# KyanChen/RSPrompter

Measured on NVIDIA H100. Metric: images/sec, higher is better.
Workload: dtype bf16

## Files before the change

include/rsp_b200.h:

```cpp
#ifndef RSP_B200_H_
#define RSP_B200_H_

#include <stdint.h>

#ifdef __cplusplus
extern "C" {
#endif

#define RSP_ABI_VERSION 2

int rsp_abi_version(void);
const char* rsp_last_error(void);

int rsp_gemm_bf16(const void* A, int lda, const void* W, int ldw, void* out, int ldo, int M, int N,
                  int K, const float* bias, const void* residual, int ldr, int res_fp32, int res_mod,
                  const int32_t* row_map, int act, int out_fp32, void* stream);

int rsp_conv3x3_nhwc_bf16(const void* x, int B, int H, int W, int C, const void* Wt, int ldw, void* out, int ldo,
                          int N, const float* bias, const void* residual, int ldr, int res_fp32, int act,
                          int out_fp32, void* stream);
int rsp_conv3x3_geometry_ok(int B, int H, int W, int C);

int rsp_gemm_bf16_simt(const void* A, int lda, const void* W, int ldw, void* out, int ldo, int M,
                       int N, int K, const float* bias, const void* residual, int ldr, int res_fp32,
                       int res_mod, const int32_t* row_map, int act, int out_fp32, void* stream);

int rsp_vit_attention(const void* qkv, const void* rel_h, const void* rel_w, void* out, int n_seq,
                      int T, int S, int H, int hd, void* stream);
int rsp_vit_attention_scatter(const void* qkv, const void* rel_h, const void* rel_w, void* out, int n_seq, int T,
                              int Sg, int H, int hd, const int32_t* out_row_map, void* stream);

int rsp_vit_attention_simt(const void* qkv, const void* rel_h, const void* rel_w, void* out,
                           int n_seq, int T, int S, int H, int hd, void* stream);

int rsp_layernorm(const void* in, int in_fp32, int ld_in, void* out, int out_fp32, int ld_out,
                  const float* gamma, const float* beta, const int32_t* src_map, int rows_out, int C,
                  float eps, int act, void* copy_out, int ld_copy, void* stream);

int rsp_layernorm_add(const void* x, const void* res, int res_fp32, const int32_t* res_block_map,
                      int res_block_rows, const float* gamma, const float* beta, void* out, const float* pos,
                      int pos_mod, void* out_pe, long long rows, int C, float eps, void* stream);

int rsp_patchify16(const float* img, void* out, int B, int H, int W, void* stream);

int rsp_im2col_nhwc(const void* in, void* out, int B, int H, int W, int C, int KH, int KW,
                    int stride, int pad, void* stream);

int rsp_nhwc_to_nchw(const void* in, int in_fp32, float* out, int B, int HW, int C, void* stream);

int rsp_gemm_bf16_ex(const void* A, int lda, const void* W, int ldw, void* out, int ldo, int M, int N,
                     int K, const float* bias, const void* residual, int ldr, int res_fp32, int res_mod,
                     const int32_t* row_map, int act, int out_fp32, int epi_mode, const float* ln_gamma,
                     const float* ln_beta, float ln_eps, const int32_t* res_block_map,
                     int res_block_rows, const float* hyper, float* mask_out, int grid_h, int grid_w,
                     void* stream);

int rsp_gemm_upscale_masks(const void* A, int lda, const void* W, int ldw, int M, int K, const float* bias,
                           const float* hyper, int n_out, float* mask_out, int grid_h, int grid_w, void* stream);

int rsp_add_cast_bf16(const float* a, const float* b, void* out, long long n, long long b_mod,
                      void* stream);

int rsp_token_self_attention(const void* q, const void* k, const void* v, void* out, int N, int T,
                             int heads, int c, void* stream);
int rsp_t2i_attention(const void* q, const void* K, const void* V, int ldkv, const int32_t* kv_block, void* out,
                      int N, int Tq, int HW, void* stream);
// ... 153 lines not shown
```

rsprompter_b200/_lib.py:

```python
from __future__ import annotations

import ctypes
import os
import subprocess
from pathlib import Path

import torch

_PKG_DIR = Path(__file__).resolve().parent
LIB_PATH = _PKG_DIR / "librsp_b200.so"
CSRC_DIR = _PKG_DIR / "csrc"


class RspError(RuntimeError):
    """Raised when an ``rsp_*`` entry point returns a non-zero status."""


def build_library(verbose: bool = False) -> Path:
    cmd = ["make", "-C", str(CSRC_DIR), "-j", str(os.cpu_count() or 4), "all"]
    res = subprocess.run(cmd, capture_output=True, text=True)
    if res.returncode != 0:
        raise RuntimeError(f"building librsp_b200.so failed:\n{res.stdout[-4000:]}\n{res.stderr[-4000:]}")
    if verbose:
        print(res.stdout[-2000:])
    return LIB_PATH


def _load() -> ctypes.CDLL:
    if not LIB_PATH.exists():
        raise ImportError(
            f"{LIB_PATH} not found: the CUDA extension is mandatory (no fallback path). "
            "Run `python -c 'import __graft_entry__ as g; g.build()'` or `make -C rsprompter_b200/csrc`.")
    return ctypes.CDLL(str(LIB_PATH))


_lib = _load()

_vp, _i, _f = ctypes.c_void_p, ctypes.c_int, ctypes.c_float

_SIGNATURES = {
    "rsp_abi_version": ([], _i),
    "rsp_last_error": ([], ctypes.c_char_p),
    "rsp_gemm_bf16": ([_vp, _i, _vp, _i, _vp, _i, _i, _i, _i, _vp, _vp, _i, _i, _i, _vp, _i, _i, _vp], _i),
    "rsp_gemm_bf16_simt": ([_vp, _i, _vp, _i, _vp, _i, _i, _i, _i, _vp, _vp, _i, _i, _i, _vp, _i, _i, _vp], _i),
    "rsp_vit_attention": ([_vp, _vp, _vp, _vp, _i, _i, _i, _i, _i, _vp], _i),
    "rsp_vit_attention_scatter": ([_vp, _vp, _vp, _vp, _i, _i, _i, _i, _i, _vp, _vp], _i),
    "rsp_vit_attention_simt": ([_vp, _vp, _vp, _vp, _i, _i, _i, _i, _i, _vp], _i),
    "rsp_layernorm": ([_vp, _i, _i, _vp, _i, _i, _vp, _vp, _vp, _i, _i, _f, _i, _vp, _i, _vp], _i),
    "rsp_patchify16": ([_vp, _vp, _i, _i, _i, _vp], _i),
    "rsp_layernorm_add": ([_vp, _vp, _i, _vp, _i, _vp, _vp, _vp, _vp, _i, _vp, ctypes.c_longlong, _i, _f, _vp], _i),
    "rsp_im2col_nhwc": ([_vp, _vp, _i, _i, _i, _i, _i, _i, _i, _i, _vp], _i),
    "rsp_nhwc_to_nchw": ([_vp, _i, _vp, _i, _i, _i, _vp], _i),
    "rsp_cast_f32_bf16": ([_vp, _vp, ctypes.c_longlong, _vp], _i),
    "rsp_add_table_bf16": ([_vp, _vp, _vp, ctypes.c_longlong, ctypes.c_longlong, _vp], _i),
    "rsp_gemm_bf16_ex": ([_vp, _i, _vp, _i, _vp, _i, _i, _i, _i, _vp, _vp, _i, _i, _i, _vp, _i, _i,
                          _i, _vp, _vp, _f, _vp, _i, _vp, _vp, _i, _i, _vp], _i),
    "rsp_add_cast_bf16": ([_vp, _vp, _vp, ctypes.c_longlong, ctypes.c_longlong, _vp], _i),
    "rsp_token_self_attention": ([_vp, _vp, _vp, _vp, _i, _i, _i, _i, _vp], _i),
    "rsp_t2i_attention": ([_vp, _vp, _vp, _i, _vp, _vp, _i, _i, _i, _vp], _i),
    "rsp_i2t_attention": ([_vp, _vp, _vp, _vp, _vp, _i, _i, _i, _vp], _i),
    "rsp_t2i_fused": ([_vp, _i, _vp, _vp, _vp, _vp, _vp, _i, _i, _i, _vp], _i),
    "rsp_i2t_fused": ([_vp, _i, _vp, _vp, _vp, _vp, _vp, _vp, _vp, _vp, _vp, _f, _vp, _i, _i, _i, _vp], _i),
    "rsp_rpn_decode": ([_vp, _i, _vp, _i, _i, _i, _i, _i, _i, _vp, _vp, _f, _f, _f, _i, _i, _vp, _vp, _vp], _i),
    "rsp_bbox_cls_decode": ([_vp, _i, _vp, _i, _vp, _vp, _i, _i, _vp, _f, _f, _f, _vp, _vp, _vp, _vp], _i),
    "rsp_rpn_decode_shapes": ([_vp, _i, _vp, _i, _i, _i, _i, _i, _i, _vp, _vp, _vp, _f, _i, _i, _vp, _vp, _vp], _i),
    "rsp_nms_batched_topk": ([_vp, _vp, _vp, _i, _i, _f, _vp, _vp, _vp, _i, _vp], _i),
    "rsp_bbox_cls_decode_shapes": ([_vp, _i, _vp, _i, _vp, _vp, _i, _i, _vp, _vp, _f, _vp, _vp, _vp, _vp], _i),
    "rsp_nms_batched": ([_vp, _vp, _vp, _i, _i, _f, _vp, _vp, _vp, _vp], _i),
    "rsp_compact_keep": ([_vp, _vp, _vp, _vp, _i, _i, _i, _vp, _vp, _vp, _vp, _vp, _vp], _i),
    "rsp_soft_nms_workspace_bytes": ([_i, _i, _i, _vp], _i),
    "rsp_soft_nms_batched": ([_vp, _vp, _vp, _vp, _i, _i, _i, _f, _f, _f, _i, _i, _i, _vp, ctypes.c_size_t, _vp, _vp,
                              _vp, _vp, _vp, _vp], _i),
    "rsp_roi_align_nhwc": ([_vp, _vp, _vp, _vp, _vp, _i, _vp, _i, _i, _i, _f, _vp, _vp], _i),
    "rsp_mask_paste": ([_vp, _vp, _i, _i, _i, _i, _i, _f, _i, _vp], _i),
    "rsp_pool2_nhwc": ([_vp, _vp, _i, _i, _i, _i, _i, _vp], _i),
    "rsp_zero_border_nhwc": ([_vp, _i, _i, _i, _i, _vp], _i),
    "rsp_sigmoid_f32": ([_vp, _vp, ctypes.c_longlong, _vp], _i),
    "rsp_mask_paste_boxes": ([_vp, _vp, _vp, _i, _i, _i, _i, _i, _f, _i, _vp], _i),
    "rsp_groupnorm_nhwc": ([_vp, _vp, _vp, _vp, _vp, _vp, _i, _i, _i, _i, _i, _f, _i, _vp], _i),
    "rsp_ms_deform_attn_sample": ([_vp, _vp, _i, _vp, _vp, _i, _i, _i, _i, _vp, _vp], _i),
# ... 1146 lines not shown
```

rsprompter_b200/csrc/abi.cu:

```cuda
#include "../../include/rsp_b200.h"

#include "attention.h"
#include "gemm.h"
#include "rowops.h"

namespace rsp { const char* last_error(); }
using namespace rsp;

static inline cudaStream_t S(void* s) { return static_cast<cudaStream_t>(s); }

extern "C" {

int rsp_abi_version(void) { return RSP_ABI_VERSION; }
const char* rsp_last_error(void) { return rsp::last_error(); }

static GemmArgs make_gemm_args(const void* A, int lda, const void* W, int ldw, void* out, int ldo,
                               int M, int N, int K, const float* bias, const void* residual, int ldr,
                               int res_fp32, int res_mod, const int32_t* row_map, int act,
                               int out_fp32) {
  GemmArgs a;
  a.A = A; a.lda = lda; a.W = W; a.ldw = ldw; a.out = out; a.ldo = ldo;
  a.M = M; a.N = N; a.K = K; a.bias = bias; a.residual = residual; a.ldr = ldr;
  a.res_fp32 = res_fp32; a.res_mod = res_mod; a.row_map = row_map; a.act = act;
  a.out_fp32 = out_fp32;
// ... 23 lines not shown
  return conv3x3_bf16(a, S(stream));
}

int rsp_conv3x3_geometry_ok(int B, int H, int W, int C) { return conv3x3_geometry_ok(B, H, W, C) ? 1 : 0; }

int rsp_gemm_bf16_simt(const void* A, int lda, const void* W, int ldw, void* out, int ldo, int M,
                       int N, int K, const float* bias, const void* residual, int ldr, int res_fp32,
                       int res_mod, const int32_t* row_map, int act, int out_fp32, void* stream) {
  return gemm_bf16_simt(make_gemm_args(A, lda, W, ldw, out, ldo, M, N, K, bias, residual, ldr,
                                       res_fp32, res_mod, row_map, act, out_fp32), S(stream));
}

static AttentionArgs make_att_args(const void* qkv, const void* rel_h, const void* rel_w, void* out,
                                   int n_seq, int T, int Sg, int H, int hd, const int32_t* out_row_map = nullptr) {
  AttentionArgs a;
  a.qkv = qkv; a.rel_h = rel_h; a.rel_w = rel_w; a.out = out;
  a.n_seq = n_seq; a.T = T; a.S = Sg; a.H = H; a.hd = hd; a.out_row_map = out_row_map;
  return a;
}

int rsp_vit_attention(const void* qkv, const void* rel_h, const void* rel_w, void* out, int n_seq,
                      int T, int Sg, int H, int hd, void* stream) {
  return vit_attention(make_att_args(qkv, rel_h, rel_w, out, n_seq, T, Sg, H, hd), S(stream));
}

int rsp_vit_attention_scatter(const void* qkv, const void* rel_h, const void* rel_w, void* out, int n_seq, int T,
                              int Sg, int H, int hd, const int32_t* out_row_map, void* stream) {
  return vit_attention(make_att_args(qkv, rel_h, rel_w, out, n_seq, T, Sg, H, hd, out_row_map), S(stream));
}

int rsp_vit_attention_simt(const void* qkv, const void* rel_h, const void* rel_w, void* out,
                           int n_seq, int T, int Sg, int H, int hd, void* stream) {
  return vit_attention_simt(make_att_args(qkv, rel_h, rel_w, out, n_seq, T, Sg, H, hd), S(stream));
}

int rsp_attn_softmax_bias(const float* scores, int lds, const float* tab, int ldt, int NT, void* P, int ldp, int n_rows,
                          int T, int Sg, float scale, void* stream) {
  return attn_softmax_bias(scores, lds, tab, ldt, NT, P, ldp, n_rows, T, Sg, scale, S(stream));
}

int rsp_transpose_cols(const void* in, int ld, int col0, int C, int n_seq, int T, void* out, void* stream) {
  return transpose_cols(in, ld, col0, C, n_seq, T, out, S(stream));
}

int rsp_split_heads(const void* in, int ld, int col0, int H, int hd, int n_seq, int T, void* out, void* stream) {
  return split_heads(in, ld, col0, H, hd, n_seq, T, out, S(stream));
}

int rsp_layernorm(const void* in, int in_fp32, int ld_in, void* out, int out_fp32, int ld_out,
                  const float* gamma, const float* beta, const int32_t* src_map, int rows_out, int C,
                  float eps, int act, void* copy_out, int ld_copy, void* stream) {
  LayerNormArgs a;
  a.copy_out = copy_out; a.ld_copy = ld_copy;
  a.in = in; a.in_fp32 = in_fp32; a.ld_in = ld_in; a.out = out; a.out_fp32 = out_fp32;
  a.ld_out = ld_out; a.gamma = gamma; a.beta = beta; a.src_map = src_map; a.rows_out = rows_out;
  a.C = C; a.eps = eps; a.act = act;
  return layernorm_rows(a, S(stream));
}

int rsp_layernorm_add(const void* x, const void* res, int res_fp32, const int32_t* res_block_map,
                      int res_block_rows, const float* gamma, const float* beta, void* out, const float* pos,
                      int pos_mod, void* out_pe, long long rows, int C, float eps, void* stream) {
  return layernorm_add(x, res, res_fp32, res_block_map, res_block_rows, gamma, beta, out, pos, pos_mod, out_pe, rows,
                       C, eps, S(stream));
}

// ... 344 lines not shown
```

rsprompter_b200/csrc/attention.cu:

```cuda
#include <cstdlib>

#include "attention.h"
#include "sm90.cuh"

namespace rsp {

constexpr float LOG2E = 1.4426950408889634f;

__device__ __forceinline__ float fast_exp2(float x) {
  float y;
  asm("ex2.approx.ftz.f32 %0, %1;" : "=f"(y) : "f"(x));
  return y;
}
__device__ __forceinline__ uint32_t pack_f16x2(float lo, float hi) {
  __half2 v = __floats2half2_rn(lo, hi);
  return *reinterpret_cast<uint32_t*>(&v);
}
__device__ __forceinline__ uint32_t bf16x2_to_f16x2(uint32_t w) {
  return pack_f16x2(__uint_as_float(w << 16), __uint_as_float(w & 0xffff0000u));
}

template <int HD, int S>
struct AttCfg {
  static constexpr int T = S * S;
// ... 344 lines not shown
  const uint64_t tstr[1] = {static_cast<uint64_t>(HD) * 2};
  const uint32_t qbox[3] = {64, C::BM, 1}, qbox_t[3] = {16, C::BM, 1};
  const uint32_t kvbox[3] = {64, C::BN, 1}, kvbox_t[3] = {16, C::BN, 1};
  const uint32_t tbox[2] = {64, static_cast<uint32_t>(C::NTAB)}, tbox_t[2] = {16, static_cast<uint32_t>(C::NTAB)};
  CUtensorMap tq, tkv, th, tw, tq_t, tkv_t, th_t, tw_t;
  RSP_TRY(make_tmap_swizzled(&tq, a.qkv, 3, qdims, qstr, qbox, 0, 128));
  RSP_TRY(make_tmap_swizzled(&tkv, a.qkv, 3, qdims, qstr, kvbox, 0, 128));
  RSP_TRY(make_tmap_swizzled(&th, a.rel_h, 2, tdims, tstr, tbox, 0, 128));
  RSP_TRY(make_tmap_swizzled(&tw, a.rel_w, 2, tdims, tstr, tbox, 0, 128));
  if (C::TAIL > 0) {
    RSP_TRY(make_tmap_swizzled(&tq_t, a.qkv, 3, qdims, qstr, qbox_t, 0, 32));
    RSP_TRY(make_tmap_swizzled(&tkv_t, a.qkv, 3, qdims, qstr, kvbox_t, 0, 32));
    RSP_TRY(make_tmap_swizzled(&th_t, a.rel_h, 2, tdims, tstr, tbox_t, 0, 32));
    RSP_TRY(make_tmap_swizzled(&tw_t, a.rel_w, 2, tdims, tstr, tbox_t, 0, 32));
  } else {
    tq_t = tq; tkv_t = tkv; th_t = th; tw_t = tw;
  }
  auto kern = vit_attention_kernel<HD, S>;
  static bool attr_set_dev[kMaxDevices] = {};
  bool& attr_set = attr_set_dev[current_device()];
  if (!attr_set) {
    RSP_CHECK_CUDA(cudaFuncSetAttribute(kern, cudaFuncAttributeMaxDynamicSharedMemorySize, C::SMEM_BYTES));
    attr_set = true;
  }
  const long long items = static_cast<long long>(a.n_seq) * a.H * C::NQT;
  RSP_CHECK_ARG(items > 0 && items < (1ll << 31), "attention: %lld query tiles", items);
  p.n_items = static_cast<int>(items);
  const int grid = static_cast<int>(items < num_sms() ? items : num_sms());
  kern<<<grid, 384, C::SMEM_BYTES, stream>>>(tq, tq_t, tkv, tkv_t, th, th_t, tw, tw_t, p);
  RSP_CHECK_LAUNCH();
  return RSP_OK;
}

int vit_attention(const AttentionArgs& a, cudaStream_t stream) {
  RSP_CHECK_ARG(a.qkv && a.rel_h && a.rel_w && a.out, "attention: null pointer");
  RSP_CHECK_ARG(a.T == a.S * a.S, "attention: T=%d is not S^2 (S=%d)", a.T, a.S);
  RSP_CHECK_ARG(a.n_seq > 0 && a.H > 0, "attention: bad n_seq/H");
  if (a.S != 14 && a.S != 32 && a.S != 64)
    return vit_attention_simt(a, stream);
  if (a.hd == 64) {
    if (a.S == 64) return launch_att<64, 64>(a, stream);
    if (a.S == 32) return launch_att<64, 32>(a, stream);
    return launch_att<64, 14>(a, stream);
  }
  if (a.hd == 80) {
    if (a.S == 64) return launch_att<80, 64>(a, stream);
    if (a.S == 32) return launch_att<80, 32>(a, stream);
    return launch_att<80, 14>(a, stream);
  }
  set_last_error("attention: head dim %d unsupported (64, 80)", a.hd);
  return RSP_ERR_UNSUPPORTED;
}

__global__ void vit_attention_simt_kernel(const __nv_bfloat16* __restrict__ qkv,
                                          const __nv_bfloat16* __restrict__ rel_h,
                                          const __nv_bfloat16* __restrict__ rel_w,
                                          __nv_bfloat16* __restrict__ out, int T, int S, int H,
                                          int hd, float scale, const int* __restrict__ out_row_map) {
  const int D = H * hd;
  const int tq = blockIdx.x * blockDim.x + threadIdx.x;
  const int head = blockIdx.y;
  const int seq = blockIdx.z;
  if (tq >= T) return;
  const int qh = tq / S, qw = tq % S;
  const __nv_bfloat16* qp = qkv + (static_cast<size_t>(seq) * T + tq) * 3 * D + head * hd;
  float q[128];
  for (int d = 0; d < hd; ++d) q[d] = __bfloat162float(qp[d]);
  float rh[128], rw[128];
  for (int k = 0; k < S; ++k) {
    float ah = 0.f, aw = 0.f;
    const __nv_bfloat16* th = rel_h + static_cast<size_t>(qh - k + S - 1) * hd;
    const __nv_bfloat16* tw = rel_w + static_cast<size_t>(qw - k + S - 1) * hd;
    for (int d = 0; d < hd; ++d) {
      ah += q[d] * __bfloat162float(th[d]);
      aw += q[d] * __bfloat162float(tw[d]);
    }
    rh[k] = ah; rw[k] = aw;
  }
  float m = -INFINITY, l = 0.f;
  float o[128];
  for (int d = 0; d < hd; ++d) o[d] = 0.f;
  for (int k = 0; k < T; ++k) {
// ... 33 lines not shown
```

rsprompter_b200/csrc/attention.h:

```cpp
#pragma once
#include "host_util.h"

namespace rsp {

struct AttentionArgs {
  const void* qkv = nullptr;
  const void* rel_h = nullptr;
  const void* rel_w = nullptr;
  void* out = nullptr;
  int n_seq = 0;
  int T = 0;
  int S = 0;
  int H = 0;
  int hd = 0;
  const int* out_row_map = nullptr;
};

int vit_attention(const AttentionArgs& a, cudaStream_t stream);
int vit_attention_simt(const AttentionArgs& a, cudaStream_t stream);
int attn_softmax_bias(const float* scores, int lds, const float* tab, int ldt, int NT, void* P, int ldp, int n_rows,
                      int T, int S, float scale, cudaStream_t stream);
int transpose_cols(const void* in, int ld, int col0, int C, int n_seq, int T, void* out, cudaStream_t stream);
int split_heads(const void* in, int ld, int col0, int H, int hd, int n_seq, int T, void* out, cudaStream_t stream);

}
```

rsprompter_b200/csrc/selftest_attn.cu:

```cuda
#include <math.h>
#include <stdio.h>
#include <stdlib.h>
#include <string.h>

#include <vector>

#include "attention.h"

namespace rsp { const char* last_error(); }
using namespace rsp;

#define CK(x)                                                                        \
  do {                                                                               \
    cudaError_t e = (x);                                                             \
    if (e != cudaSuccess) {                                                          \
      printf("CUDA error %s at %s:%d\n", cudaGetErrorString(e), __FILE__, __LINE__); \
      exit(2);                                                                       \
    }                                                                                \
  } while (0)

static uint32_t a_seed = 777;
static float arand() {
  a_seed = a_seed * 1664525u + 1013904223u;
  return ((a_seed >> 8) & 0xffff) / 65536.0f - 0.5f;
// ... 8 lines not shown
  uint32_t u = (uint32_t)h << 16;
  float f;
  memcpy(&f, &u, 4);
  return f;
}

static int attn_case(const char* name, int n_seq, int S, int H, int hd, float qk_mag, float tab_mag,
                     int bench) {
  const int T = S * S, D = H * hd;
  const size_t m_tok = (size_t)n_seq * T;
  std::vector<uint16_t> hqkv(m_tok * 3 * D), hrh((size_t)(2 * S - 1) * hd), hrw((size_t)(2 * S - 1) * hd);
  for (auto& x : hqkv) x = f2bf(arand() * qk_mag);
  for (auto& x : hrh) x = f2bf(arand() * tab_mag);
  for (auto& x : hrw) x = f2bf(arand() * tab_mag);
  void *dqkv, *drh, *drw, *do1, *do2;
  CK(cudaMalloc(&dqkv, hqkv.size() * 2));
  CK(cudaMalloc(&drh, hrh.size() * 2));
  CK(cudaMalloc(&drw, hrw.size() * 2));
  CK(cudaMalloc(&do1, m_tok * D * 2));
  CK(cudaMalloc(&do2, m_tok * D * 2));
  CK(cudaMemcpy(dqkv, hqkv.data(), hqkv.size() * 2, cudaMemcpyHostToDevice));
  CK(cudaMemcpy(drh, hrh.data(), hrh.size() * 2, cudaMemcpyHostToDevice));
  CK(cudaMemcpy(drw, hrw.data(), hrw.size() * 2, cudaMemcpyHostToDevice));
  CK(cudaMemset(do1, 0xff, m_tok * D * 2));
  CK(cudaMemset(do2, 0xff, m_tok * D * 2));
  AttentionArgs a;
  a.qkv = dqkv; a.rel_h = drh; a.rel_w = drw; a.n_seq = n_seq; a.T = T; a.S = S; a.H = H; a.hd = hd;
  a.out = do1;
  int s = vit_attention(a, 0);
  if (s) { printf("[%s] vit_attention failed: %s\n", name, last_error()); return 1; }
  cudaError_t e = cudaDeviceSynchronize();
  if (e != cudaSuccess) { printf("[%s] kernel error: %s\n", name, cudaGetErrorString(e)); exit(3); }
  int fail = 0;
  if (!bench) {
    a.out = do2;
    s = vit_attention_simt(a, 0);
    if (s) { printf("[%s] simt failed: %s\n", name, last_error()); return 1; }
    CK(cudaDeviceSynchronize());
    std::vector<uint16_t> h1(m_tok * D), h2(m_tok * D);
    CK(cudaMemcpy(h1.data(), do1, h1.size() * 2, cudaMemcpyDeviceToHost));
    CK(cudaMemcpy(h2.data(), do2, h2.size() * 2, cudaMemcpyDeviceToHost));
    double maxerr = 0, maxref = 0;
    size_t nbad = 0, first_bad = (size_t)-1;
    for (size_t i = 0; i < h2.size(); ++i) if (fabs(bf2f(h2[i])) > maxref) maxref = fabs(bf2f(h2[i]));
    for (size_t i = 0; i < h1.size(); ++i) {
      const float x = bf2f(h1[i]), y = bf2f(h2[i]);
      const double d = fabs((double)x - (double)y);
      if (!(d <= 1.5e-2 * maxref)) { if (!nbad) first_bad = i; ++nbad; }
      if (d > maxerr || d != d) maxerr = d;
      if (fabs(y) > maxref) maxref = fabs(y);
    }
    printf("[%s] n_seq=%d S=%d H=%d hd=%d  max|diff|=%.3e max|ref|=%.3e bad=%zu/%zu %s\n", name,
           n_seq, S, H, hd, maxerr, maxref, nbad, h1.size(), nbad ? "FAIL" : "PASS");
    if (nbad) {
      const size_t row = first_bad / D, col = first_bad % D;
      printf("   first bad at token %zu (seq %zu, t %zu) col %zu: got %.4f want %.4f\n", row, row / T,
             row % T, col, bf2f(h1[first_bad]), bf2f(h2[first_bad]));
      for (int rr = 0; rr < 3; ++rr) {
        printf("   tok %d:", rr * 77);
        for (int j = 0; j < 6; ++j)
          printf(" %.4f/%.4f", bf2f(h1[(size_t)rr * 77 * D + j]), bf2f(h2[(size_t)rr * 77 * D + j]));
        printf("\n");
      }
      fail = 1;
    }
  } else {
    for (int i = 0; i < 3; ++i) vit_attention(a, 0);
    CK(cudaDeviceSynchronize());
    cudaEvent_t e0, e1;
    cudaEventCreate(&e0); cudaEventCreate(&e1);
    const int iters = 10;
    cudaEventRecord(e0);
    for (int i = 0; i < iters; ++i) vit_attention(a, 0);
    cudaEventRecord(e1);
    CK(cudaDeviceSynchronize());
    float ms;
    cudaEventElapsedTime(&ms, e0, e1);
    ms /= iters;
    const double flops = 4.0 * n_seq * H * (double)T * T * hd;
    printf("bench attn [%s] n_seq=%d S=%d H=%d hd=%d: %.3f ms  %.1f TFLOP/s (QK^T+PV)\n", name, n_seq,
           S, H, hd, ms, flops / ms * 1e-9);
  }
  cudaFree(dqkv); cudaFree(drh); cudaFree(drw); cudaFree(do1); cudaFree(do2);
  return fail;
}

int selftest_attention(int bench) {
  int fails = 0;
  fails += attn_case("win-hd64", 3, 14, 2, 64, 2.0f, 1.0f, 0);
  fails += attn_case("win-hd80", 3, 14, 2, 80, 2.0f, 1.0f, 0);
  fails += attn_case("win-hd64-many", 50, 14, 12, 64, 3.0f, 2.0f, 0);
  fails += attn_case("glob-hd64", 1, 64, 2, 64, 2.0f, 1.0f, 0);
  fails += attn_case("glob-hd80", 1, 64, 2, 80, 2.0f, 1.0f, 0);
  fails += attn_case("glob-hd64-sharp", 2, 64, 3, 64, 6.0f, 3.0f, 0);
  fails += attn_case("glob32-hd80", 3, 32, 2, 80, 2.0f, 1.0f, 0);
  fails += attn_case("win-hd80-sharp", 7, 14, 3, 80, 6.0f, 3.0f, 0);
  if (bench) {
    attn_case("vitb-window", 200, 14, 12, 64, 2.0f, 1.0f, 1);
    attn_case("vitb-global", 8, 64, 12, 64, 2.0f, 1.0f, 1);
    attn_case("vith-window", 200, 14, 16, 80, 2.0f, 1.0f, 1);
    attn_case("vith-global", 8, 64, 16, 80, 2.0f, 1.0f, 1);
  }
  return fails;
}
```

rsprompter_b200/csrc/sm90.cuh:

```cuda
#pragma once
#include <cuda.h>
#include <cuda_bf16.h>
#include <cuda_runtime.h>
#include <stdint.h>

namespace rsp {

__device__ __forceinline__ uint32_t smem_u32(const void* p) {
  return static_cast<uint32_t>(__cvta_generic_to_shared(p));
}

__device__ __forceinline__ uint32_t elect_one() {
  uint32_t pred = 0;
  asm volatile(
      "{\n"
      ".reg .b32 rx;\n"
      ".reg .pred px;\n"
      "elect.sync rx|px, 0xffffffff;\n"
      "selp.u32 %0, 1, 0, px;\n"
      "}\n"
      : "=r"(pred));
  return pred;
}

// ... 73 lines not shown
__device__ __forceinline__ void bulk_wait_read1() { asm volatile("cp.async.bulk.wait_group.read 1;" ::: "memory"); }
__device__ __forceinline__ void bulk_wait0() { asm volatile("cp.async.bulk.wait_group 0;" ::: "memory"); }

__device__ __forceinline__ uint64_t make_gdesc(uint32_t saddr, uint32_t lbo_bytes, uint32_t sbo_bytes) {
  uint64_t d = 0;
  d |= static_cast<uint64_t>((saddr & 0x3ffff) >> 4);
  d |= static_cast<uint64_t>((lbo_bytes >> 4) & 0x3fff) << 16;
  d |= static_cast<uint64_t>((sbo_bytes >> 4) & 0x3fff) << 32;
  d |= 1ull << 62;
  return d;
}

__device__ __forceinline__ uint64_t make_gdesc_sw32(uint32_t saddr, uint32_t lbo_bytes, uint32_t sbo_bytes) {
  uint64_t d = 0;
  d |= static_cast<uint64_t>((saddr & 0x3ffff) >> 4);
  d |= static_cast<uint64_t>((lbo_bytes >> 4) & 0x3fff) << 16;
  d |= static_cast<uint64_t>((sbo_bytes >> 4) & 0x3fff) << 32;
  d |= 3ull << 62;
  return d;
}

__device__ __forceinline__ void wgmma_fence() { asm volatile("wgmma.fence.sync.aligned;" ::: "memory"); }
__device__ __forceinline__ void wgmma_commit() { asm volatile("wgmma.commit_group.sync.aligned;" ::: "memory"); }
template <int N>
__device__ __forceinline__ void wgmma_wait() { asm volatile("wgmma.wait_group.sync.aligned %0;" ::"n"(N) : "memory"); }
template <int R>
__device__ __forceinline__ void acc_fence(float (&d)[R]) {
#pragma unroll
  for (int i = 0; i < R; ++i) asm volatile("" : "+f"(d[i])::"memory");
}

template <int N>
struct Wgmma;
template <> struct Wgmma<32> {
  template <int TB>
  __device__ __forceinline__ static void ss(float (&d)[16], uint64_t a, uint64_t b, uint32_t acc) {
    asm volatile(
        "{\n.reg .pred p;\n"
        "setp.ne.b32 p, %18, 0;\n"
        "wgmma.mma_async.sync.aligned.m64n32k16.f32.bf16.bf16 "
        "{" 
        "%0, %1, %2, %3, %4, %5, %6, %7, %8, %9, %10, %11, %12, %13, %14, %15"
        "}, %16, %17, p, 1, 1, 0, %19;\n}\n"
        : "+f"(d[0]), "+f"(d[1]), "+f"(d[2]), "+f"(d[3]), "+f"(d[4]), "+f"(d[5]), "+f"(d[6]), "+f"(d[7]),
          "+f"(d[8]), "+f"(d[9]), "+f"(d[10]), "+f"(d[11]), "+f"(d[12]), "+f"(d[13]), "+f"(d[14]), "+f"(d[15])
        : "l"(a), "l"(b), "r"(acc), "n"(TB));
  }
};
template <> struct Wgmma<64> {
  template <int TB>
  __device__ __forceinline__ static void ss(float (&d)[32], uint64_t a, uint64_t b, uint32_t acc) {
    asm volatile(
        "{\n.reg .pred p;\n"
        "setp.ne.b32 p, %34, 0;\n"
        "wgmma.mma_async.sync.aligned.m64n64k16.f32.bf16.bf16 "
        "{" 
        "%0, %1, %2, %3, %4, %5, %6, %7, %8, %9, %10, %11, %12, %13, %14, %15, "
        "%16, %17, %18, %19, %20, %21, %22, %23, %24, %25, %26, %27, %28, %29, %30, %31"
        "}, %32, %33, p, 1, 1, 0, %35;\n}\n"
        : "+f"(d[0]), "+f"(d[1]), "+f"(d[2]), "+f"(d[3]), "+f"(d[4]), "+f"(d[5]), "+f"(d[6]), "+f"(d[7]),
          "+f"(d[8]), "+f"(d[9]), "+f"(d[10]), "+f"(d[11]), "+f"(d[12]), "+f"(d[13]), "+f"(d[14]), "+f"(d[15]),
          "+f"(d[16]), "+f"(d[17]), "+f"(d[18]), "+f"(d[19]), "+f"(d[20]), "+f"(d[21]), "+f"(d[22]), "+f"(d[23]),
          "+f"(d[24]), "+f"(d[25]), "+f"(d[26]), "+f"(d[27]), "+f"(d[28]), "+f"(d[29]), "+f"(d[30]), "+f"(d[31])
        : "l"(a), "l"(b), "r"(acc), "n"(TB));
  }
};
// ... 229 lines not shown
```

Before: 58.90.

## Add persistent warp-specialized window attention kernel with shared K/V across query tiles

Replaces the per-query-tile window attention (S=14) with a persistent, warp-specialized kernel. Producer warps load each window-head's K and V once via TMA into double-buffered shared memory, and helper warps convert V to fp16 in place. Two consumer warpgroups then process all four query tiles against those shared K/V, overlapping QK^T, softmax and PV wgmmas and using an m64n8 wgmma for the 196-key tail. The previous kernel stays available as a qtile entry point for comparison. The cost is much higher kernel complexity and heavy shared-memory and register use.

New measurement: 60.18, median of 6. +2.2%, better.

```diff
diff --git a/include/rsp_b200.h b/include/rsp_b200.h
--- a/include/rsp_b200.h
+++ b/include/rsp_b200.h
@@ -32,6 +32,8 @@
 
 int rsp_vit_attention_simt(const void* qkv, const void* rel_h, const void* rel_w, void* out,
                            int n_seq, int T, int S, int H, int hd, void* stream);
+int rsp_vit_attention_qtile(const void* qkv, const void* rel_h, const void* rel_w, void* out, int n_seq, int T,
+                            int S, int H, int hd, const int32_t* out_row_map, void* stream);
 
 int rsp_layernorm(const void* in, int in_fp32, int ld_in, void* out, int out_fp32, int ld_out,
                   const float* gamma, const float* beta, const int32_t* src_map, int rows_out, int C,
diff --git a/rsprompter_b200/_lib.py b/rsprompter_b200/_lib.py
--- a/rsprompter_b200/_lib.py
+++ b/rsprompter_b200/_lib.py
@@ -46,6 +46,7 @@
     "rsp_vit_attention": ([_vp, _vp, _vp, _vp, _i, _i, _i, _i, _i, _vp], _i),
     "rsp_vit_attention_scatter": ([_vp, _vp, _vp, _vp, _i, _i, _i, _i, _i, _vp, _vp], _i),
     "rsp_vit_attention_simt": ([_vp, _vp, _vp, _vp, _i, _i, _i, _i, _i, _vp], _i),
+    "rsp_vit_attention_qtile": ([_vp, _vp, _vp, _vp, _i, _i, _i, _i, _i, _vp, _vp], _i),
     "rsp_layernorm": ([_vp, _i, _i, _vp, _i, _i, _vp, _vp, _vp, _i, _i, _f, _i, _vp, _i, _vp], _i),
     "rsp_patchify16": ([_vp, _vp, _i, _i, _i, _vp], _i),
     "rsp_layernorm_add": ([_vp, _vp, _i, _vp, _i, _vp, _vp, _vp, _vp, _i, _vp, ctypes.c_longlong, _i, _f, _vp], _i),
diff --git a/rsprompter_b200/csrc/abi.cu b/rsprompter_b200/csrc/abi.cu
--- a/rsprompter_b200/csrc/abi.cu
+++ b/rsprompter_b200/csrc/abi.cu
@@ -79,6 +79,11 @@
 int rsp_vit_attention_simt(const void* qkv, const void* rel_h, const void* rel_w, void* out,
                            int n_seq, int T, int Sg, int H, int hd, void* stream) {
   return vit_attention_simt(make_att_args(qkv, rel_h, rel_w, out, n_seq, T, Sg, H, hd), S(stream));
+}
+
+int rsp_vit_attention_qtile(const void* qkv, const void* rel_h, const void* rel_w, void* out, int n_seq, int T,
+                            int Sg, int H, int hd, const int32_t* out_row_map, void* stream) {
+  return vit_attention_qtile(make_att_args(qkv, rel_h, rel_w, out, n_seq, T, Sg, H, hd, out_row_map), S(stream));
 }
 
 int rsp_attn_softmax_bias(const float* scores, int lds, const float* tab, int ldt, int NT, void* P, int ldp, int n_rows,
diff --git a/rsprompter_b200/csrc/attention.cu b/rsprompter_b200/csrc/attention.cu
--- a/rsprompter_b200/csrc/attention.cu
+++ b/rsprompter_b200/csrc/attention.cu
@@ -400,22 +400,434 @@
   return RSP_OK;
 }
 
-int vit_attention(const AttentionArgs& a, cudaStream_t stream) {
+namespace window {
+
+template <int HD>
+struct WinCfg {
+  static constexpr int S = 14, T = S * S;
+  static constexpr int BN = 64;
+  static constexpr int NKT = (T + BN - 1) / BN;
+  static constexpr int LAST = 16;
+  static constexpr int NREL = 2 * S - 1, NTAB = 32;
+  static constexpr int TAIL = HD - 64;
+  static constexpr int SP = S + 4;
+  __host__ __device__ static constexpr int tile_bytes(int rows) { return rows * (128 + 2 * TAIL); }
+  static constexpr int TILE = tile_bytes(BN);
+  static constexpr int TILE_LAST = tile_bytes(LAST);
+  static constexpr int TILE_LAST_PAD = (TILE_LAST + 1023) / 1024 * 1024;
+  static constexpr int TILE_TAB = tile_bytes(NTAB);
+  static constexpr int K_LAST = 2 * (NKT - 1) * TILE, V_LAST = K_LAST + TILE_LAST_PAD;
+  static constexpr int KV_BYTES = V_LAST + TILE_LAST_PAD;
+  static constexpr int KV_TX = (NKT - 1) * TILE + TILE_LAST;
+  static constexpr int KVBUF = 2;
+  static constexpr int QST = 4;
+  static constexpr int BIAS_WG = 2 * BN * SP;
+  static constexpr int KV_OFF = 0;
+  static constexpr int Q_OFF = KV_OFF + KVBUF * KV_BYTES;
+  static constexpr int TAB_OFF = Q_OFF + QST * TILE;
+  static constexpr int BIAS_OFF = TAB_OFF + 2 * TILE_TAB;
+  static constexpr int BAR_OFF = BIAS_OFF + 2 * BIAS_WG * 4;
+  static constexpr int SMEM_BYTES = BAR_OFF + 8 * 32 + 1024;
+  static constexpr int REG_PRODUCER = 40, REG_CONSUMER = 232;
+  static_assert(HD == 64 || HD == 80, "head dim");
+  static_assert(NKT == 4 && T > (NKT - 1) * BN && T <= (NKT - 1) * BN + 8, "the last tile's keys fit one N = 8 wgmma");
+  static_assert(TILE % 1024 == 0 && TILE_TAB % 1024 == 0 && KV_BYTES % 1024 == 0, "swizzle atoms");
+  static_assert(1 + 4 * KVBUF + 2 * QST <= 32, "barriers");
+  static_assert(SMEM_BYTES <= 227 * 1024, "shared memory");
+};
+
+template <int N, int TAIL>
+__device__ __forceinline__ void qk_issue(float (&acc)[N / 2], uint32_t qa, uint32_t qtail, uint32_t b, int b_rows) {
+  acc_fence(acc);
+  wgmma_fence();
+#pragma unroll
+  for (int k = 0; k < 4; ++k)
+    Wgmma<N>::template ss<0>(acc, make_gdesc(qa + 32 * k, 16, 1024), make_gdesc(b + 32 * k, 16, 1024), k);
+  if constexpr (TAIL > 0)
+    Wgmma<N>::template ss<0>(acc, make_gdesc_sw32(qtail, 16, 256), make_gdesc_sw32(b + b_rows * 128, 16, 256), 1);
+  wgmma_commit();
+}
+
+template <int J, int NS, int NKK>
+__device__ __forceinline__ void window_softmax(float (&sc)[NS], int r0, int cq, float scale2, const float* relh,
+                                               const float (&rw)[2][14], float (&m_run)[2], float (&l_run)[2],
+                                               float (&alpha)[2], uint32_t (&pa)[NKK][4]) {
+  constexpr int S = 14, T = S * S, BN = 64, SP = S + 4, NKT = (T + BN - 1) / BN;
+  constexpr int A0 = J * BN / S, A1 = (J * BN + 8 * (NS / 4 - 1) + 1) / S + 1, NH = A1 - A0 + 1;
+  static_assert(A1 < SP, "rel_h row");
+  int c = cq;
+  asm volatile("" : "+r"(c));
+  float hh[2][NH];
+#pragma unroll
+  for (int i = 0; i < 2; ++i)
+#pragma unroll
+    for (int a = 0; a < NH; ++a) hh[i][a] = relh[(r0 + 8 * i) * SP + A0 + a];
+  float mx[2] = {-INFINITY, -INFINITY};
+#pragma unroll
+  for (int x = 0; x < NS; ++x) {
+    const int i = (x >> 1) & 1;
+    const int k0 = J * BN + 8 * (x >> 2) + (x & 1);
+    const int a = k0 / S - A0, m = k0 % S;
+    float t = -INFINITY;
+    if (J < NKT - 1 || k0 + c < T) {
+      const bool w = m + c >= S;
+      t = fmaf(sc[x], scale2, (w ? hh[i][a + 1] : hh[i][a]) + rw[i][m]);
+    }
+    sc[x] = t;
+    mx[i] = fmaxf(mx[i], t);
+  }
+#pragma unroll
+  for (int i = 0; i < 2; ++i) {
+    mx[i] = fmaxf(mx[i], __shfl_xor_sync(0xffffffffu, mx[i], 1));
+    mx[i] = fmaxf(mx[i], __shfl_xor_sync(0xffffffffu, mx[i], 2));
+    const float m_new = fmaxf(m_run[i], mx[i]);
+    alpha[i] = fast_exp2(m_run[i] - m_new);
+    m_run[i] = m_new;
+    l_run[i] *= alpha[i];
+  }
+#pragma unroll
+  for (int kk = 0; kk < NKK; ++kk) {
+#pragma unroll
+    for (int h = 0; h < 4; ++h) {
+      const int x = 8 * kk + 2 * h, i = h & 1;
+      if (x < NS) {
+        const float p0 = fast_exp2(sc[x] - m_run[i]), p1 = fast_exp2(sc[x + 1] - m_run[i]);
+        l_run[i] += p0 + p1;
+        pa[kk][h] = pack_f16x2(p0, p1);
+      } else {
+        pa[kk][h] = 0u;
+      }
+    }
+  }
+}
+
+template <int NKK, int TAIL>
+__device__ __forceinline__ void window_pv(float (&om)[32], float (&ot)[8], const float (&alpha)[2],
+                                          const uint32_t (&pa)[NKK][4], uint32_t vb, int v_rows) {
+  acc_fence(om);
+  acc_fence(ot);
+#pragma unroll
+  for (int y = 0; y < 32; ++y) om[y] *= alpha[(y >> 1) & 1];
+#pragma unroll
+  for (int y = 0; y < 8; ++y) ot[y] *= alpha[(y >> 1) & 1];
+  wgmma_fence();
+#pragma unroll
+  for (int kk = 0; kk < NKK; ++kk) {
+    WgmmaRsF16<64>::rs(om, pa[kk], make_gdesc(vb + kk * 2048, 64 * 128, 1024));
+    if constexpr (TAIL > 0) WgmmaRsF16<16>::rs(ot, pa[kk], make_gdesc_sw32(vb + v_rows * 128 + kk * 512, 256, 256));
+  }
+  wgmma_commit();
+}
+
+template <int HD, int S>
+__global__ void __launch_bounds__(384, 1)
+vit_attention_kernel(const __grid_constant__ CUtensorMap tm_x, const __grid_constant__ CUtensorMap tm_x_t,
+                     const __grid_constant__ CUtensorMap tm_xl, const __grid_constant__ CUtensorMap tm_xl_t,
+                     const __grid_constant__ CUtensorMap tm_rh, const __grid_constant__ CUtensorMap tm_rh_t,
+                     const __grid_constant__ CUtensorMap tm_rw, const __grid_constant__ CUtensorMap tm_rw_t,
+                     const AttDev p) {
+  static_assert(S == 14, "windows only");
+  using C = WinCfg<HD>;
+  constexpr int T = C::T, BN = C::BN, NKT = C::NKT, SP = C::SP, TAIL = C::TAIL, QST = C::QST, KVBUF = C::KVBUF;
+  constexpr int LAST = C::LAST;
+  constexpr uint32_t TILE = C::TILE, TILE_TAB = C::TILE_TAB;
+  extern __shared__ __align__(1024) uint8_t smem_raw[];
+  uint8_t* smem = smem_raw + ((1024u - (smem_u32(smem_raw) & 1023u)) & 1023u);
+  const uint32_t sbase = smem_u32(smem);
+  uint64_t* bar_tab = reinterpret_cast<uint64_t*>(smem + C::BAR_OFF);
+  uint64_t* bar_k = bar_tab + 1;
+  uint64_t* bar_v = bar_k + KVBUF;
+  uint64_t* bar_vc = bar_v + KVBUF;
+  uint64_t* bar_kve = bar_vc + KVBUF;
+  uint64_t* bar_q = bar_kve + KVBUF;
+  uint64_t* bar_qe = bar_q + QST;
+
+  const int warp = threadIdx.x >> 5, lane = threadIdx.x & 31;
+  if (threadIdx.x == 0) {
+    tma_prefetch_desc(&tm_x);
+    mbar_init(smem_u32(bar_tab), 1);
+    for (int b = 0; b < KVBUF; ++b) {
+      mbar_init(smem_u32(&bar_k[b]), 1);
+      mbar_init(smem_u32(&bar_v[b]), 1);
+      mbar_init(smem_u32(&bar_vc[b]), 3);
+      mbar_init(smem_u32(&bar_kve[b]), 8);
+    }
+    for (int s = 0; s < QST; ++s) {
+      mbar_init(smem_u32(&bar_q[s]), 1);
+      mbar_init(smem_u32(&bar_qe[s]), 4);
+    }
+    fence_barrier_init();
+  }
+  __syncthreads();
+
+  if (warp < 4) {
+    setmaxnreg_dec<C::REG_PRODUCER>();
+    if (warp == 0) {
+      if (lane == 0) {
+        const uint32_t bq = smem_u32(bar_tab);
+        mbar_expect_tx(bq, 2 * TILE_TAB);
+        tma_load_2d(sbase + C::TAB_OFF, &tm_rh, bq, 0, 0);
+        tma_load_2d(sbase + C::TAB_OFF + TILE_TAB, &tm_rw, bq, 0, 0);
+        if constexpr (TAIL > 0) {
+          tma_load_2d(sbase + C::TAB_OFF + C::NTAB * 128, &tm_rh_t, bq, 64, 0);
+          tma_load_2d(sbase + C::TAB_OFF + TILE_TAB + C::NTAB * 128, &tm_rw_t, bq, 64, 0);
+        }
+#pragma unroll 1
+        for (int item = blockIdx.x, it = 0; item < p.n_items; item += gridDim.x, ++it) {
+          const int head = item % p.H, seq = item / p.H;
+          const int colq = head * HD, colk = p.D + colq, colv = 2 * p.D + colq;
+          const int b = it % KVBUF;
+          mbar_wait(smem_u32(&bar_kve[b]), ((it / KVBUF) & 1) ^ 1);
+          const uint32_t kvb = sbase + C::KV_OFF + b * C::KV_BYTES;
+#pragma unroll 1
+          for (int kv = 0; kv < 2; ++kv) {
+            const uint32_t bar = smem_u32(kv ? &bar_v[b] : &bar_k[b]);
+            const int col = kv ? colv : colk;
+            mbar_expect_tx(bar, C::KV_TX);
+#pragma unroll 1
+            for (int j = 0; j < NKT - 1; ++j)
+              load_tile<TAIL>(kvb + (kv * (NKT - 1) + j) * TILE, BN, &tm_x, &tm_x_t, bar, col, j * BN, seq);
+            load_tile<TAIL>(kvb + (kv ? C::V_LAST : C::K_LAST), LAST, &tm_xl, &tm_xl_t, bar, col, (NKT - 1) * BN,
+                            seq);
+          }
+#pragma unroll 1
+          for (int sl = 0; sl < NKT; ++sl) {
+            const int gq = it * NKT + sl, s = gq % QST;
+            mbar_wait(smem_u32(&bar_qe[s]), ((gq / QST) & 1) ^ 1);
+            mbar_expect_tx(smem_u32(&bar_q[s]), TILE);
+            load_tile<TAIL>(sbase + C::Q_OFF + s * TILE, BN, &tm_x, &tm_x_t, smem_u32(&bar_q[s]), colq, sl * BN, seq);
+          }
+        }
+      }
+    } else {
+      const int t = threadIdx.x - 32;
+#pragma unroll 1
+      for (int item = blockIdx.x, it = 0; item < p.n_items; item += gridDim.x, ++it) {
+        const int b = it % KVBUF;
+        mbar_wait(smem_u32(&bar_v[b]), (it / KVBUF) & 1);
+        uint8_t* kvs = smem + C::KV_OFF + b * C::KV_BYTES;
+#pragma unroll 1
+        for (int part = 0; part < 2; ++part) {
+          uint4* v = reinterpret_cast<uint4*>(kvs + (part ? C::V_LAST : (NKT - 1) * TILE));
+          const int n = (part ? C::TILE_LAST : (NKT - 1) * TILE) / 16;
+#pragma unroll 4
+          for (int i = t; i < n; i += 96) {
+            uint4 w = v[i];
+            w.x = bf16x2_to_f16x2(w.x);
+            w.y = bf16x2_to_f16x2(w.y);
+            w.z = bf16x2_to_f16x2(w.z);
+            w.w = bf16x2_to_f16x2(w.w);
+            v[i] = w;
+          }
+        }
+        fence_proxy_async_smem();
+        __syncwarp();
+        if (lane == 0) mbar_arrive(smem_u32(&bar_vc[b]));
+      }
+    }
+    return;
+  }
+
+  setmaxnreg_inc<C::REG_CONSUMER>();
+  const int wg = (warp >> 2) - 1;
+  const int r0 = (warp & 3) * 16 + (lane >> 2);
+  const int cq = 2 * (lane & 3);
+  float* relh = reinterpret_cast<float*>(smem + C::BIAS_OFF) + wg * C::BIAS_WG;
+  float* relw = relh + BN * SP;
+  const float scale2 = p.scale2;
+  mbar_wait(smem_u32(bar_tab), 0);
+#pragma unroll 1
+  for (int item = blockIdx.x, it = 0; item < p.n_items; item += gridDim.x, ++it) {
+    const int head = item % p.H, seq = item / p.H;
+    const int b = it % KVBUF;
+    const uint32_t kph = (it / KVBUF) & 1;
+    const uint32_t kvb = sbase + C::KV_OFF + b * C::KV_BYTES;
+    const uint32_t vb = kvb + (NKT - 1) * TILE;
+#pragma unroll 1
+    for (int sl = wg; sl < NKT; sl += 2) {
+      const int gq = it * NKT + sl, s = gq % QST;
+      const uint32_t qa = sbase + C::Q_OFF + s * TILE;
+      const uint32_t qtail = qa + BN * 128;
+
+      mbar_wait(smem_u32(&bar_q[s]), (gq / QST) & 1);
+      named_bar_sync(1 + wg, 128);
+      float tabs[2][C::NTAB / 2];
+      qk_issue<C::NTAB, TAIL>(tabs[0], qa, qtail, sbase + C::TAB_OFF, C::NTAB);
+      qk_issue<C::NTAB, TAIL>(tabs[1], qa, qtail, sbase + C::TAB_OFF + TILE_TAB, C::NTAB);
+      float s0[BN / 2], s1[BN / 2], s2[BN / 2], s3[4];
+      mbar_wait(smem_u32(&bar_k[b]), kph);
+      qk_issue<BN, TAIL>(s0, qa, qtail, kvb, BN);
+#pragma unroll
+      for (int tab = 0; tab < 2; ++tab) {
+        if (tab == 0) wgmma_wait<2>(); else wgmma_wait<1>();
+        acc_fence(tabs[tab]);
+        float* dst = tab ? relw : relh;
+#pragma unroll
+        for (int x = 0; x < C::NTAB / 2; ++x) {
+          const int r = r0 + 8 * ((x >> 1) & 1);
+          const int tq = sl * BN + r;
+          const int qc = tab ? tq % S : tq / S;
+          const int t = 8 * (x >> 2) + cq + (x & 1);
+          const int k = qc + S - 1 - t;
+          if (t < C::NREL && k >= 0 && k < S) dst[r * SP + k] = tabs[tab][x] * LOG2E;
+        }
+      }
+      named_bar_sync(1 + wg, 128);
+      float rw[2][S];
+#pragma unroll
+      for (int i = 0; i < 2; ++i)
+#pragma unroll
+        for (int m = 0; m < S; ++m) {
+          const int kw = m + cq;
+          rw[i][m] = relw[(r0 + 8 * i) * SP + (kw >= S ? kw - S : kw)];
+        }
+
+      float om[32], ot[8];
+#pragma unroll
+      for (int y = 0; y < 32; ++y) om[y] = 0.f;
+#pragma unroll
+      for (int y = 0; y < 8; ++y) ot[y] = 0.f;
+      float m_run[2] = {-INFINITY, -INFINITY}, l_run[2] = {0.f, 0.f}, alpha[2];
+      uint32_t pa[BN / 16][4], pl[1][4];
+      wgmma_wait<0>();
+      acc_fence(s0);
+      qk_issue<BN, TAIL>(s1, qa, qtail, kvb + TILE, BN);
+      window_softmax<0>(s0, r0, cq, scale2, relh, rw, m_run, l_run, alpha, pa);
+      mbar_wait(smem_u32(&bar_vc[b]), kph);
+      window_pv<BN / 16, TAIL>(om, ot, alpha, pa, vb, BN);
+      wgmma_wait<1>();
+      acc_fence(s1);
+      qk_issue<BN, TAIL>(s2, qa, qtail, kvb + 2 * TILE, BN);
+      window_softmax<1>(s1, r0, cq, scale2, relh, rw, m_run, l_run, alpha, pa);
+      wgmma_wait<1>();
+      window_pv<BN / 16, TAIL>(om, ot, alpha, pa, vb + TILE, BN);
+      wgmma_wait<1>();
+      acc_fence(s2);
+      qk_issue<8, TAIL>(s3, qa, qtail, kvb + C::K_LAST, LAST);
+      window_softmax<2>(s2, r0, cq, scale2, relh, rw, m_run, l_run, alpha, pa);
+      wgmma_wait<1>();
+      window_pv<BN / 16, TAIL>(om, ot, alpha, pa, vb + 2 * TILE, BN);
+      wgmma_wait<1>();
+      acc_fence(s3);
+      __syncwarp();
+      if (lane == 0) mbar_arrive(smem_u32(&bar_qe[s]));
+      window_softmax<NKT - 1>(s3, r0, cq, scale2, relh, rw, m_run, l_run, alpha, pl);
+      wgmma_wait<0>();
+      window_pv<1, TAIL>(om, ot, alpha, pl, kvb + C::V_LAST, LAST);
+      wgmma_wait<0>();
+      acc_fence(om);
+      acc_fence(ot);
+      if (sl + 2 >= NKT) {
+        __syncwarp();
+        if (lane == 0) mbar_arrive(smem_u32(&bar_kve[b]));
+      }
+
+#pragma unroll
+      for (int i = 0; i < 2; ++i) {
+        float l = l_run[i];
+        l += __shfl_xor_sync(0xffffffffu, l, 1);
+        l += __shfl_xor_sync(0xffffffffu, l, 2);
+        const float inv = 1.0f / l;
+        const int tq = sl * BN + r0 + 8 * i;
+        if (tq >= T) continue;
+        int dst = seq * T + tq;
+        if (p.out_row_map) dst = __ldg(p.out_row_map + dst);
+        if (dst < 0) continue;
+        __nv_bfloat16* orow = p.out + static_cast<size_t>(dst) * p.D + head * HD + cq;
+#pragma unroll
+        for (int nb = 0; nb < 8; ++nb)
+          *reinterpret_cast<uint32_t*>(orow + nb * 8) = pack_bf16x2(om[4 * nb + 2 * i] * inv, om[4 * nb + 2 * i + 1] * inv);
+        if constexpr (TAIL > 0) {
+#pragma unroll
+          for (int nb = 0; nb < 2; ++nb)
+            *reinterpret_cast<uint32_t*>(orow + 64 + nb * 8) =
+                pack_bf16x2(ot[4 * nb + 2 * i] * inv, ot[4 * nb + 2 * i + 1] * inv);
+        }
+      }
+    }
+  }
+}
+
+}
+
+template <int HD>
+static int launch_window(const AttentionArgs& a, cudaStream_t stream) {
+  using C = window::WinCfg<HD>;
+  RSP_CHECK_ARG((reinterpret_cast<uintptr_t>(a.qkv) & 15) == 0 && (reinterpret_cast<uintptr_t>(a.rel_h) & 15) == 0 &&
+                (reinterpret_cast<uintptr_t>(a.rel_w) & 15) == 0 && (reinterpret_cast<uintptr_t>(a.out) & 3) == 0,
+                "attention: qkv / tables must be 16-byte aligned");
+  AttDev p;
+  p.out = static_cast<__nv_bfloat16*>(a.out);
+  p.out_row_map = a.out_row_map;
+  p.H = a.H; p.D = a.H * HD;
+  p.scale2 = (1.0f / sqrtf(static_cast<float>(HD))) * LOG2E;
+  const uint64_t ld = 3ull * p.D;
+  const uint64_t xdims[3] = {ld, static_cast<uint64_t>(C::T), static_cast<uint64_t>(a.n_seq)};
+  const uint64_t xstr[2] = {ld * 2, ld * 2 * C::T};
+  const uint64_t tdims[2] = {static_cast<uint64_t>(HD), static_cast<uint64_t>(C::NREL)};
+  const uint64_t tstr[1] = {static_cast<uint64_t>(HD) * 2};
+  const uint32_t xbox[3] = {64, C::BN, 1}, xbox_t[3] = {16, C::BN, 1};
+  const uint32_t lbox[3] = {64, C::LAST, 1}, lbox_t[3] = {16, C::LAST, 1};
+  const uint32_t tbox[2] = {64, static_cast<uint32_t>(C::NTAB)}, tbox_t[2] = {16, static_cast<uint32_t>(C::NTAB)};
+  CUtensorMap tx, tl, th, tw, tx_t, tl_t, th_t, tw_t;
+  RSP_TRY(make_tmap_swizzled(&tx, a.qkv, 3, xdims, xstr, xbox, 0, 128));
+  RSP_TRY(make_tmap_swizzled(&tl, a.qkv, 3, xdims, xstr, lbox, 0, 128));
+  RSP_TRY(make_tmap_swizzled(&th, a.rel_h, 2, tdims, tstr, tbox, 0, 128));
+  RSP_TRY(make_tmap_swizzled(&tw, a.rel_w, 2, tdims, tstr, tbox, 0, 128));
+  if (C::TAIL > 0) {
+    RSP_TRY(make_tmap_swizzled(&tx_t, a.qkv, 3, xdims, xstr, xbox_t, 0, 32));
+    RSP_TRY(make_tmap_swizzled(&tl_t, a.qkv, 3, xdims, xstr, lbox_t, 0, 32));
+    RSP_TRY(make_tmap_swizzled(&th_t, a.rel_h, 2, tdims, tstr, tbox_t, 0, 32));
+    RSP_TRY(make_tmap_swizzled(&tw_t, a.rel_w, 2, tdims, tstr, tbox_t, 0, 32));
+  } else {
+    tx_t = tx; tl_t = tl; th_t = th; tw_t = tw;
+  }
+  auto kern = window::vit_attention_kernel<HD, C::S>;
+  static bool attr_set_dev[kMaxDevices] = {};
+  bool& attr_set = attr_set_dev[current_device()];
+  if (!attr_set) {
+    RSP_CHECK_CUDA(cudaFuncSetAttribute(kern, cudaFuncAttributeMaxDynamicSharedMemorySize, C::SMEM_BYTES));
+    attr_set = true;
+  }
+  const long long items = static_cast<long long>(a.n_seq) * a.H;
+  RSP_CHECK_ARG(items > 0 && items < (1ll << 31), "attention: %lld (window, head) items", items);
+  p.n_items = static_cast<int>(items);
+  const int grid = static_cast<int>(items < num_sms() ? items : num_sms());
+  kern<<<grid, 384, C::SMEM_BYTES, stream>>>(tx, tx_t, tl, tl_t, th, th_t, tw, tw_t, p);
+  RSP_CHECK_LAUNCH();
+  return RSP_OK;
+}
+
+static int check_att_args(const AttentionArgs& a) {
   RSP_CHECK_ARG(a.qkv && a.rel_h && a.rel_w && a.out, "attention: null pointer");
   RSP_CHECK_ARG(a.T == a.S * a.S, "attention: T=%d is not S^2 (S=%d)", a.T, a.S);
   RSP_CHECK_ARG(a.n_seq > 0 && a.H > 0, "attention: bad n_seq/H");
+  return RSP_OK;
+}
+
+int vit_attention(const AttentionArgs& a, cudaStream_t stream) {
+  RSP_TRY(check_att_args(a));
   if (a.S != 14 && a.S != 32 && a.S != 64)
     return vit_attention_simt(a, stream);
   if (a.hd == 64) {
     if (a.S == 64) return launch_att<64, 64>(a, stream);
     if (a.S == 32) return launch_att<64, 32>(a, stream);
-    return launch_att<64, 14>(a, stream);
+    return launch_window<64>(a, stream);
   }
   if (a.hd == 80) {
     if (a.S == 64) return launch_att<80, 64>(a, stream);
     if (a.S == 32) return launch_att<80, 32>(a, stream);
-    return launch_att<80, 14>(a, stream);
-  }
+    return launch_window<80>(a, stream);
+  }
+  set_last_error("attention: head dim %d unsupported (64, 80)", a.hd);
+  return RSP_ERR_UNSUPPORTED;
+}
+
+int vit_attention_qtile(const AttentionArgs& a, cudaStream_t stream) {
+  RSP_TRY(check_att_args(a));
+  RSP_CHECK_ARG(a.S == 14, "attention_qtile: S=%d (windows only)", a.S);
+  if (a.hd == 64) return launch_att<64, 14>(a, stream);
+  if (a.hd == 80) return launch_att<80, 14>(a, stream);
   set_last_error("attention: head dim %d unsupported (64, 80)", a.hd);
   return RSP_ERR_UNSUPPORTED;
 }
diff --git a/rsprompter_b200/csrc/attention.h b/rsprompter_b200/csrc/attention.h
--- a/rsprompter_b200/csrc/attention.h
+++ b/rsprompter_b200/csrc/attention.h
@@ -18,6 +18,7 @@
 
 int vit_attention(const AttentionArgs& a, cudaStream_t stream);
 int vit_attention_simt(const AttentionArgs& a, cudaStream_t stream);
+int vit_attention_qtile(const AttentionArgs& a, cudaStream_t stream);
 int attn_softmax_bias(const float* scores, int lds, const float* tab, int ldt, int NT, void* P, int ldp, int n_rows,
                       int T, int S, float scale, cudaStream_t stream);
 int transpose_cols(const void* in, int ld, int col0, int C, int n_seq, int T, void* out, cudaStream_t stream);
diff --git a/rsprompter_b200/csrc/selftest_attn.cu b/rsprompter_b200/csrc/selftest_attn.cu
--- a/rsprompter_b200/csrc/selftest_attn.cu
+++ b/rsprompter_b200/csrc/selftest_attn.cu
@@ -64,6 +64,19 @@
   cudaError_t e = cudaDeviceSynchronize();
   if (e != cudaSuccess) { printf("[%s] kernel error: %s\n", name, cudaGetErrorString(e)); exit(3); }
   int fail = 0;
+  if (S == 14) {
+    a.out = do2;
+    s = vit_attention_qtile(a, 0);
+    if (s) { printf("[%s] vit_attention_qtile failed: %s\n", name, last_error()); return 1; }
+    CK(cudaDeviceSynchronize());
+    std::vector<uint16_t> h1(m_tok * D), h2(m_tok * D);
+    CK(cudaMemcpy(h1.data(), do1, h1.size() * 2, cudaMemcpyDeviceToHost));
+    CK(cudaMemcpy(h2.data(), do2, h2.size() * 2, cudaMemcpyDeviceToHost));
+    const bool same = memcmp(h1.data(), h2.data(), h1.size() * 2) == 0;
+    printf("[%s] window kernel vs query-tile kernel: %s\n", name, same ? "bytes identical" : "BYTES DIFFER FAIL");
+    if (!same) return 1;
+    a.out = do1;
+  }
   if (!bench) {
     a.out = do2;
     s = vit_attention_simt(a, 0);
@@ -97,21 +110,29 @@
       fail = 1;
     }
   } else {
-    for (int i = 0; i < 3; ++i) vit_attention(a, 0);
+    const int n_arms = S == 14 ? 2 : 1, rounds = S == 14 ? 5 : 1, iters = 10;
+    int (*const arms[2])(const AttentionArgs&, cudaStream_t) = {vit_attention, vit_attention_qtile};
+    const char* arm_name[2] = {"", " query-tile kernel"};
+    for (int k = 0; k < n_arms; ++k)
+      for (int i = 0; i < 3; ++i) arms[k](a, 0);
     CK(cudaDeviceSynchronize());
     cudaEvent_t e0, e1;
     cudaEventCreate(&e0); cudaEventCreate(&e1);
-    const int iters = 10;
-    cudaEventRecord(e0);
-    for (int i = 0; i < iters; ++i) vit_attention(a, 0);
-    cudaEventRecord(e1);
-    CK(cudaDeviceSynchronize());
-    float ms;
-    cudaEventElapsedTime(&ms, e0, e1);
-    ms /= iters;
+    float best[2] = {1e30f, 1e30f};
+    for (int r = 0; r < rounds; ++r)
+      for (int k = 0; k < n_arms; ++k) {
+        cudaEventRecord(e0);
+        for (int i = 0; i < iters; ++i) arms[k](a, 0);
+        cudaEventRecord(e1);
+        CK(cudaDeviceSynchronize());
+        float ms;
+        cudaEventElapsedTime(&ms, e0, e1);
+        if (ms / iters < best[k]) best[k] = ms / iters;
+      }
     const double flops = 4.0 * n_seq * H * (double)T * T * hd;
-    printf("bench attn [%s] n_seq=%d S=%d H=%d hd=%d: %.3f ms  %.1f TFLOP/s (QK^T+PV)\n", name, n_seq,
-           S, H, hd, ms, flops / ms * 1e-9);
+    for (int k = 0; k < n_arms; ++k)
+      printf("bench attn [%s%s] n_seq=%d S=%d H=%d hd=%d: %.3f ms  %.1f TFLOP/s (QK^T+PV)\n", name, arm_name[k],
+             n_seq, S, H, hd, best[k], flops / best[k] * 1e-9);
   }
   cudaFree(dqkv); cudaFree(drh); cudaFree(drw); cudaFree(do1); cudaFree(do2);
   return fail;
diff --git a/rsprompter_b200/csrc/sm90.cuh b/rsprompter_b200/csrc/sm90.cuh
--- a/rsprompter_b200/csrc/sm90.cuh
+++ b/rsprompter_b200/csrc/sm90.cuh
@@ -129,6 +129,18 @@
 
 template <int N>
 struct Wgmma;
+template <> struct Wgmma<8> {
+  template <int TB>
+  __device__ __forceinline__ static void ss(float (&d)[4], uint64_t a, uint64_t b, uint32_t acc) {
+    asm volatile(
+        "{\n.reg .pred p;\n"
+        "setp.ne.b32 p, %6, 0;\n"
+        "wgmma.mma_async.sync.aligned.m64n8k16.f32.bf16.bf16 "
+        "{%0, %1, %2, %3}, %4, %5, p, 1, 1, 0, %7;\n}\n"
+        : "+f"(d[0]), "+f"(d[1]), "+f"(d[2]), "+f"(d[3])
+        : "l"(a), "l"(b), "r"(acc), "n"(TB));
+  }
+};
 template <> struct Wgmma<32> {
   template <int TB>
   __device__ __forceinline__ static void ss(float (&d)[16], uint64_t a, uint64_t b, uint32_t acc) {
```
